# l646773422/h264-lab

Measured on AMD Instinct MI355X. Metric: 1080p macroblocks/sec, higher is better.
Workload: dtype u8

## Files before the change

h264-lab_amd/csrc/enc_kernels.h:

```cpp
#ifndef H264E_ENC_KERNELS_H
#define H264E_ENC_KERNELS_H

#include "wave.h"
#include "tables.h"
#include "h264e_dev.h"

#define MV_NA H264E_MV_NA
#define NNZ_NA 64
#define AV_T 1
#define AV_L 2
#define AV_TL 4
#define AV_TR 8
#define QMODE_I4 2
#define QMODE_INTER 8
#define QMODE_I16 9
#define QMODE_CHROMA 5
#define QD_RND 6
#define QD_THR1 10
#define QD_THR2 18
#define MUL_LAMBDA(x, l) ((x)*(l) >> 4)

DEV int mvx(mv32 v) { return (int16_t)(v & 0xffff); }
DEV int mvy(mv32 v) { return (int16_t)((uint32_t)v >> 16); }
DEV mv32 mvmk(int x, int y) { return (mv32)(((uint32_t)y << 16) | ((uint32_t)x & 0xffff)); }
DEV mv32 mvadd(mv32 a, mv32 b) { return mvmk(mvx(a) + mvx(b), mvy(a) + mvy(b)); }
DEV mv32 mvsub(mv32 a, mv32 b) { return mvmk(mvx(a) - mvx(b), mvy(a) - mvy(b)); }
DEV mv32 mvround(mv32 a) { return mvmk((mvx(a) + 1) & ~3, (mvy(a) + 1) & ~3); }

struct qblk_t { int16_t qv[16]; int16_t dq[16]; };

struct RowTask
{
    int slice_type, qp, speed, no_deblock, narrow, nslices, frame_slot;
    const uint8_t *in[3];
    int in_stride[3];
    const uint8_t *ref[3];
    uint8_t *dec[3];
    const int *dep_progress;
    mv32 clusters[2];
    const mv32 *clusters_per_mb;
};
DEV RowTask rowtask_load(const h264e_frame_task_t &T)
{
    RowTask t;
    t.slice_type = uni(T.slice_type); t.qp = uni(T.qp); t.speed = uni(T.speed); t.no_deblock = uni(T.no_deblock); t.narrow = uni(T.narrow);
    t.nslices = uni(T.nslices); t.frame_slot = uni(T.frame_slot);
    for (int c = 0; c < 3; c++) { t.in[c] = uniptr(T.in[c]); t.in_stride[c] = uni(T.in_stride[c]); t.ref[c] = uniptr(T.ref[c]); t.dec[c] = uniptr(T.dec[c]); }
    t.dep_progress = uniptr(T.dep_progress);
    t.clusters[0] = (mv32)uni(T.clusters[0]); t.clusters[1] = (mv32)uni(T.clusters[1]);
    t.clusters_per_mb = uniptr(T.clusters_per_mb);
    return t;
}


struct BitW
{
    uint64_t acc;
    int nacc;
    uint32_t pos;
    uint32_t cap;
    int overflow;
    GLOBAL_AS uint32_t *buf;
};

DEV void bw_put(BitW &b, int n, uint32_t v)
{
    n = uni(n); v = (uint32_t)uni((int)v);
    b.acc = (b.acc << n) | (uint64_t)v;
    b.nacc += n;
    if (b.nacc >= 32)
    {
        b.nacc -= 32;
        if (b.pos < b.cap) cstore32((gu8 *)(b.buf + b.pos), (uint32_t)(b.acc >> b.nacc));
        else b.overflow = 1;
        b.pos++;
        b.acc &= (1ull << b.nacc) - 1;
    }
}
DEV BitW bw_uniform(const BitW &s)
{
    BitW b;
    b.acc = (uint64_t)(uint32_t)uni((int)(uint32_t)s.acc) | ((uint64_t)(uint32_t)uni((int)(uint32_t)(s.acc >> 32)) << 32);
    b.nacc = uni(s.nacc); b.pos = (uint32_t)uni((int)s.pos); b.cap = (uint32_t)uni((int)s.cap); b.overflow = uni(s.overflow);
    b.buf = uniptr(s.buf);
    return b;
}
DEV int ue_len(uint32_t v) { return 2*(32 - clz32(v + 1)) - 1; }
DEV void bw_ue(BitW &b, uint32_t v)
{
    int n = ue_len(v);
    if (n > 32) { bw_put(b, n - 32, 0); n = 32; }
    bw_put(b, n, v + 1);
}
DEV void bw_se(BitW &b, int v) { bw_ue(b, (uint32_t)(v > 0 ? 2*v - 1 : -2*v)); }
DEV int se_len(int v) { return ue_len((uint32_t)(v > 0 ? 2*v - 1 : -2*v)); }
DEV uint32_t bw_bits(const BitW &b) { return b.pos*32u + (uint32_t)b.nacc; }


struct Plane { const gu8 *p; int w, h, stride; };

NOINLINE_DEV uint32_t ref_load4_border(const gu8 *row, int w, int x)
{
    uint32_t v = 0;
    for (int k = 0; k < 4; k++)
    {
        const int xx = imin(imax(x + k, 0), w - 1);
        v |= ((cload32(row + (xx & ~3)) >> (8*(xx & 3))) & 255u) << (8*k);
    }
    return v;
}

DEV uint64_t cload64x2(const gu8 *p) { return (uint64_t)cload32(p) | ((uint64_t)cload32(p + 4) << 32); }

DEV uint32_t ref_load4(const Plane &P, int x, int y)
{
    y = imin(imax(y, 0), P.h - 1);
    const gu8 *r = P.p + (size_t)y*P.stride;
    if (H264E_PLAIN_UNALIGNED_LOADS && x >= 0 && x + 3 < P.w) return gload32(r + x);
    if (x >= 0 && x + 7 < P.w)
    {
        const uint64_t d = cload64x2(r + (x & ~3));
        return alignbyte32((uint32_t)(d >> 32), (uint32_t)d, (unsigned)x & 3);
    }
    return ref_load4_border(r, P.w, x);
}

DEV uint32_t lds32(const uint8_t *p) { uint32_t v; memcpy(&v, p, 4); return v; }
DEV void lds32_store(uint8_t *p, uint32_t v) { memcpy(p, &v, 4); }

DEV uint32_t lds32u(const lu8 *p)
{
    const unsigned a = (unsigned)(uintptr_t)p & 3;
    const LDS_AS uint32_t *q = (const LDS_AS uint32_t *)(p - a);
    return alignbyte32(ld32_aligned(q + 1), ld32_aligned(q), a);
}

#define WIN_M 24
#define WIN_W 64
#define WIN_STRIDE 68
struct RefView
{
    Plane P; const lu8 *win; int has_win, wx0, wy0;
    const GLOBAL_AS int *dep;
    int nmbx, nmby;
    int vw, vh;
    int *far;
    int *fail;
    const int16_t *slice_row;
    int nslices;
    unsigned spin_limit;
};

DEV bool rv_inside(const RefView &V, int x0, int y0, int x1, int y1)
{
    return V.has_win && x0 >= V.wx0 && y0 >= V.wy0 && x1 < V.wx0 + V.vw && y1 < V.wy0 + V.vh;
}
DEV const lu8 *rv_ptr(const RefView &V, int x, int y) { return V.win + (y - V.wy0)*WIN_STRIDE + (x - V.wx0); }

DEV bool rv_slice_last(const RefView &V, int Y)
{
    for (int k = 1; k <= V.nslices; k++) if (V.slice_row[k] == Y + 1) return true;
    return false;
}
DEV void rv_wait_row(const RefView &V, int drow, int need)
{
    const GLOBAL_AS int *flag = V.dep + drow;
    unsigned spins = 0;
    for (;;)
    {
        const int seen = uni(dep_poll(flag));
        if (seen >= need) break;
        if (seen < 0) { if (V.fail) *V.fail = seen; break; }
        if (++spins > V.spin_limit) { if (V.fail) *V.fail = -1; break; }
        wave_nap();
    }
}
DEV void rv_wait_rect(const RefView &V, int y0, int x1, int y1)
{
    if (V.far) *V.far += 1;
    if (!V.dep) return;
    const int X = imin(imax(x1, 0), V.P.w - 1) >> 4, Ya = imin(imax(y0, 0), V.P.h - 1) >> 4, Yb = imin(imax(y1, 0), V.P.h - 1) >> 4;
    const int need = imin(X + 2, V.nmbx);
    for (int Y = Ya; Y <= Yb; Y++)
    {
        const bool last = rv_slice_last(V, Y);
        if (last) rv_wait_row(V, Y, need);
        else if (Y == Yb) rv_wait_row(V, Y + 1, need);
    }
    consumer_acquire();
}

DEV void rv_wait_rect_g(const RefView &V, int y0, int x1, int y1)
{
    if (V.far) grp_count(V.far);
    if (!V.dep) return;
    const int X = imin(imax(x1, 0), V.P.w - 1) >> 4, Ya = imin(imax(y0, 0), V.P.h - 1) >> 4, Yb = imin(imax(y1, 0), V.P.h - 1) >> 4;
    const int need = imin(X + 2, V.nmbx);
    for (int Y = Ya; Y <= Yb; Y++)
    {
        const bool last = rv_slice_last(V, Y);
        if (!last && Y != Yb) continue;
        const GLOBAL_AS int *flag = V.dep + (last ? Y : Y + 1);
        unsigned spins = 0;
        for (;;)
        {
            const int seen = dep_poll(flag);
            if (seen >= need) break;
            if (seen < 0) { if (V.fail) *V.fail = seen; break; }
            if (++spins > V.spin_limit) { if (V.fail) *V.fail = -1; break; }
            wave_nap();
        }
    }
    consumer_acquire();
}

DEV void wave_load_window(uint8_t *win, const Plane &P, int wx0, int wy0, int narrow)
{
    const int rows = narrow ? H264E_NARROW_VH : WIN_W;
    const bool interior = wx0 >= 0 && wx0 + WIN_W <= P.w;
    if (interior)
    {
        u32x4 v[4];
        WAVE_FOR(l)
        {
            const int seg = l & 3;
#pragma unroll
            for (int k = 0; k < 4; k++)
            {
                const int r = (l >> 2) + 16*k;
                if (r < rows)
                {
                    const int y = imin(imax(wy0 + r, 0), P.h - 1);
                    v[k] = cload128(P.p + (size_t)y*P.stride + wx0 + 16*seg);
                }
            }
#pragma unroll
            for (int k = 0; k < 4; k++)
            {
                const int r = (l >> 2) + 16*k;
                if (r < rows)
                {
                    uint8_t *d = win + r*WIN_STRIDE + 16*seg;
                    lds32_store(d, v[k].x); lds32_store(d + 4, v[k].y); lds32_store(d + 8, v[k].z); lds32_store(d + 12, v[k].w);
                }
            }
        }
    } else
    {
        const int nq = narrow ? (H264E_NARROW_VW + 7)/8 : WIN_W/8;
        WAVE_FOR(l)
        {
            if (l < rows)
            {
                const int y = imin(imax(wy0 + l, 0), P.h - 1);
                for (int g = 0; g < 2*nq; g++) lds32_store(win + l*WIN_STRIDE + 4*g, ref_load4(P, wx0 + 4*g, y));
            }
        }
    }
    wave_sync();
}


DEV int wave_sad_ref(const RefView &R, int x0, int y0, const uint8_t *b, int w, int h)
{
    const int g = w >> 2, n = g*h;
    if (rv_inside(R, x0, y0, x0 + w - 1, y0 + h - 1))
    {
        const lu8 *base = rv_ptr(R, x0, y0);
        return wave_sum([&](int l) -> int {
            if (l >= n) return 0;
            int r = l >> (g >> 1), c = l & (g - 1);
            return (int)sad4_u8(lds32u(base + r*WIN_STRIDE + 4*c), lds32(b + 16*r + 4*c), 0);
        });
    }
    rv_wait_rect(R, y0, x0 + w - 1, y0 + h - 1);
    return wave_sum([&](int l) -> int {
        if (l >= n) return 0;
        int r = l >> (g >> 1), c = l & (g - 1);
        return (int)sad4_u8(ref_load4(R.P, x0 + 4*c, y0 + r), lds32(b + 16*r + 4*c), 0);
    });
}

DEV int grp_sad_ref(const RefView &R, int x0, int y0, const uint8_t *b, int w, int h)
{
    const int g = w >> 2, npass = (g*h) >> 4;
    if (rv_inside(R, x0, y0, x0 + w - 1, y0 + h - 1))
    {
        const lu8 *base = rv_ptr(R, x0, y0);
        return grp_sum([&](int i) -> int {
            uint32_t s = 0;
            for (int k = 0; k < npass; k++)
            {
                const int d = i + 16*k, r = d >> (g >> 1), c = d & (g - 1);
                s = sad4_u8(lds32u(base + r*WIN_STRIDE + 4*c), lds32(b + 16*r + 4*c), s);
            }
            return (int)s;
        });
    }
    rv_wait_rect_g(R, y0, x0 + w - 1, y0 + h - 1);
    return grp_sum([&](int i) -> int {
        uint32_t s = 0;
        for (int k = 0; k < npass; k++)
        {
            const int d = i + 16*k, r = d >> (g >> 1), c = d & (g - 1);
            s = sad4_u8(ref_load4(R.P, x0 + 4*c, y0 + r), lds32(b + 16*r + 4*c), s);
        }
        return (int)s;
    });
}

DEV int grp_sad_ref_q(const RefView &R, int x0, int y0, const uint8_t *b, int sad4[4])
{
    if (rv_inside(R, x0, y0, x0 + 15, y0 + 15))
    {
        const lu8 *base = rv_ptr(R, x0, y0);
        grp_sum4([&](int i, int *v) {
            uint32_t top = 0, bot = 0;
            const int c = i & 3;
            for (int k = 0; k < 4; k++)
            {
                const int r = (i >> 2) + 4*k;
                const uint32_t s = sad4_u8(lds32u(base + r*WIN_STRIDE + 4*c), lds32(b + 16*r + 4*c), 0);
                if (k < 2) top += s; else bot += s;
            }
            v[c >> 1] = (int)top; v[2 + (c >> 1)] = (int)bot;
        }, sad4);
    } else
    {
        rv_wait_rect_g(R, y0, x0 + 15, y0 + 15);
        grp_sum4([&](int i, int *v) {
            uint32_t top = 0, bot = 0;
            const int c = i & 3;
            for (int k = 0; k < 4; k++)
            {
                const int r = (i >> 2) + 4*k;
                const uint32_t s = sad4_u8(ref_load4(R.P, x0 + 4*c, y0 + r), lds32(b + 16*r + 4*c), 0);
                if (k < 2) top += s; else bot += s;
            }
            v[c >> 1] = (int)top; v[2 + (c >> 1)] = (int)bot;
        }, sad4);
    }
    return sad4[0] + sad4[1] + sad4[2] + sad4[3];
}

DEV int wave_sad_ref_q(const RefView &R, int x0, int y0, const uint8_t *b, int sad4[4])
{
    if (rv_inside(R, x0, y0, x0 + 15, y0 + 15))
    {
        const lu8 *base = rv_ptr(R, x0, y0);
        wave_sum4([&](int l, int *v) {
            int r = l >> 2, c = l & 3;
            v[(r >> 3)*2 + (c >> 1)] = (int)sad4_u8(lds32u(base + r*WIN_STRIDE + 4*c), lds32(b + 16*r + 4*c), 0);
        }, sad4);
    } else
    {
        rv_wait_rect(R, y0, x0 + 15, y0 + 15);
        wave_sum4([&](int l, int *v) {
            int r = l >> 2, c = l & 3;
            v[(r >> 3)*2 + (c >> 1)] = (int)sad4_u8(ref_load4(R.P, x0 + 4*c, y0 + r), lds32(b + 16*r + 4*c), 0);
        }, sad4);
    }
    return sad4[0] + sad4[1] + sad4[2] + sad4[3];
}

DEV int wave_sad_lds(const uint8_t *a, const uint8_t *b, int w, int h)
{
    const int g = w >> 2, n = g*h;
    return wave_sum([&](int l) -> int {
        if (l >= n) return 0;
        int r = l >> (g >> 1), c = l & (g - 1);
        return (int)sad4_u8(lds32(a + 16*r + 4*c), lds32(b + 16*r + 4*c), 0);
    });
}

DEV int wave_sad_lds_q(const uint8_t *a, const uint8_t *b, int sad4[4])
{
    wave_sum4([&](int l, int *v) {
        int r = l >> 2, c = l & 3;
        v[(r >> 3)*2 + (c >> 1)] = (int)sad4_u8(lds32(a + 16*r + 4*c), lds32(b + 16*r + 4*c), 0);
    }, sad4);
    return sad4[0] + sad4[1] + sad4[2] + sad4[3];
}


DEV int tap6(int a, int b, int c, int d, int e, int f) { return a - 5*b + 20*c + 20*d - 5*e + f; }
DEV int tap6w(int a, int b, int c, int d, int e, int f)
{
    const int t = (c + d)*4 - (b + e);
    return (a + f) + t*4 + t;
}

template <class LD> DEV uint32_t interp_core(LD ld, int fx, int fy)
{
    if (!(fx | fy)) return ld(0, 0);
    const int pos = fx + 4*fy;
    int A[4], B[4];
    bool avg = true;
    if (fy == 0)
    {
        const uint32_t a = ld(-4, 0), b = ld(0, 0), c = ld(4, 0);
        int p[12];
#pragma unroll
        for (int k = 0; k < 4; k++) { p[k] = (int)((a >> (8*k)) & 255); p[4 + k] = (int)((b >> (8*k)) & 255); p[8 + k] = (int)((c >> (8*k)) & 255); }
#pragma unroll
        for (int i = 0; i < 4; i++)
        {
            B[i] = clip255((tap6(p[i + 2], p[i + 3], p[i + 4], p[i + 5], p[i + 6], p[i + 7]) + 16) >> 5);
            A[i] = pos == 3 ? p[5 + i] : p[4 + i];
        }
// ... 722 lines not shown
```

h264-lab_amd/csrc/enc_mb.h:

```cpp
#ifndef H264E_ENC_MB_H
#define H264E_ENC_MB_H

#include <stddef.h>
#include "enc_kernels.h"

struct GCtx { mv32 mv_left[4], mv_tl[4], mv_top[8]; };
#define GSCR_OFF(t) ((t) == 0 ? 0 : (t) == 1 ? 1024 : (t) == 2 ? 1536 : 2048)
#define GSCR_BYTES 2304

struct MbBuf
{
    alignas(16) uint8_t inp[256];
    alignas(16) uint8_t inp_c[128];
    alignas(16) uint8_t pred[256];
    alignas(4) uint8_t pix_top[36];
    alignas(4) uint8_t ptop[96];
    mv32 mv_top[8];
    uint8_t nnz_top[8];
    int8_t i4_top[4];
    uint32_t df_nz_top;
    int top_type, top_qp;
    mv32 mv[16], mvd[16];
    int type, cost, used_cand;
    mv32 mv_skip_pred;
};

struct RowLds
{
    mv32 mv_left[4], mv_tl[4];
    uint8_t nnz_left[8];
    int8_t i4_left[4];
    alignas(4) uint8_t pix_left[32];
    uint8_t pix_tl[4];
    uint32_t df_nzflag;
    mv32 df_mv[25];
    int left_type, left_qp;
    alignas(4) uint8_t strip_y[16*4];
    alignas(4) uint8_t strip_c[2][8*4];
    alignas(4) uint8_t brec[64];
    BitW bw;
    int skip_run, lead_skips, coded_any;
    int far_reads[3];
    int far_fail[3];
    int16_t slice_row[H264E_MAX_SLICES + 2];
    unsigned long long prof[4][32], prof_last[4], prof_c0, prof_w0;
    int f_noskip, f_bound, f_inter, f_decided, f_wdone, f_stop;
    int early_bound;
    int f_t3req, f_t3done;
    int f_front, d_type[2];
    int t3_sad_best, t3_lim[4];
    mv32 t3_mv_best;

    MbBuf mb[2];
    alignas(4) uint8_t trec[72];

    int8_t i4_mode[16];
    alignas(4) uint8_t bs[32];
    I4Scratch i4s;
    uint8_t nzctx[12];
    alignas(16) uint8_t pred_c[128];
    alignas(16) uint8_t i16pred[256];
    alignas(16) uint8_t tt[256];
    alignas(16) uint8_t i4rec[17*24];
    alignas(16) uint8_t ytile[20*YT_STRIDE];
    alignas(16) uint8_t ctile[2][10*CT_STRIDE];
    alignas(16) qblk_t qy[16];
    qblk_t qu[4], qv[4];
    int16_t dcy[16], dcu[4], dcv[4], lev_dcy[16], lev_dcu[4], lev_dcv[4];

    CavlcTab cavlc;
    DfTab dftab;
    int qconst[6];
    uint16_t qdat[2][42];

    mv32 part_mv[4][4], part_mvd[4][4];
    GCtx gctx[4];
    int gcost[4], gnum[4];
    alignas(16) uint8_t win[WIN_W*WIN_STRIDE + 16];
    alignas(16) uint8_t skip_pred[256];
    alignas(16) uint8_t skip_pred_c[128];
    alignas(16) uint8_t gtest[4][256];
    alignas(16) uint8_t gscr[GSCR_BYTES];

};
#define ROWLDS_INTRA_BYTES offsetof(RowLds, part_mv)

struct MbCtx
{
    const h264e_geom_t *G;
    int speed, slice_type;
    mv32 clu[2];
    const mv32 *clu_per_mb;
    Plane ref[3];
    RefView rv;
    gu8 *dec[3];
    int x, y, num, avail, type, cost, i16_mode, cropped, used_cand;
    int slice_top;
    mv32 mv_skip_pred;
    unsigned nz_mask;
    int qp;
    int lambda_mv, lambda_q4, skip_thr, skip_thr_i4, lambda_i4, lambda_i16;
};

struct rect_t { int x0, y0, x1, y1; };

DEV int in_rect(mv32 v, const rect_t &r) { return mvy(v) >= r.y0 && mvy(v) <= r.y1 && mvx(v) >= r.x0 && mvx(v) <= r.x1; }
DEV mv32 clip_rect(mv32 v, const rect_t &r) { return mvmk(imin(imax(mvx(v), r.x0), r.x1), imin(imax(mvy(v), r.y0), r.y1)); }
DEV mv32 mb_abs(const MbCtx &m, mv32 v) { return mvadd(v, mvmk(m.x*64, m.y*64)); }
DEV int mv_cost(const MbCtx &m, mv32 v, mv32 pred)
{
    return MUL_LAMBDA(se_len(mvx(v) - mvx(pred)) + se_len(mvy(v) - mvy(pred)), m.lambda_mv);
}
DEV rect_t mv_limit(const MbCtx &m) { rect_t r = { m.G->lim_x0, m.G->lim_y0, m.G->lim_x1, m.G->lim_y1 }; return r; }
DEV rect_t mv_qlimit(const MbCtx &m) { rect_t r = { m.G->lim_x0 + 16, m.G->lim_y0 + 16, m.G->lim_x1 - 16, m.G->lim_y1 - 16 }; return r; }


DEV int med3(int a, int b, int c) { return imax(imin(imax(a, b), c), imin(a, b)); }

DEV void mvp_put_arr(mv32 *mv_left, mv32 *mv_tl, mv32 *mv_top, int x, int y, int w, int h, mv32 mv)
{
    mv_tl[y] = mv_top[x + w - 1];
    for (int i = 1; i < h; i++) mv_tl[y + i] = mv;
    for (int i = 0; i < h; i++) mv_left[y + i] = mv;
    for (int i = 0; i < w; i++) mv_top[x + i] = mv;
}
DEV void mvp_put(RowLds &L, MbBuf &B, int x, int y, int w, int h, mv32 mv) { mvp_put_arr(L.mv_left, L.mv_tl, B.mv_top, x, y, w, h, mv); }

DEV mv32 mvp_get_arr(const mv32 *mv_left, const mv32 *mv_tl, const mv32 *mv_top, int flag, int x, int y, int w, int h)
{
    int type = 1;
    mv32 a = mv_left[y], b = mv_top[x], c = mv_top[x + w], d = mv_tl[y], ret = 0;
    if (!x)
    {
        if (!(flag & AV_L)) a = MV_NA;
        if (!(flag & AV_TL)) d = MV_NA;
    }
    if (!y)
    {
        if (!(flag & AV_T))
        {
            b = MV_NA;
            if (x + w < 4) c = MV_NA;
            if (x > 0) d = MV_NA;
        }
        if (!(flag & AV_TL) && !x) d = MV_NA;
        if (!(flag & AV_TR) && x + w == 4) c = MV_NA;
    }
    if (x + w == 4 && (!(flag & AV_TR) || y)) c = d;
#define OK(v) ((v) != MV_NA)
    if (OK(a) && !OK(b) && !OK(c)) type = 2;
    else if (!OK(a) && OK(b) && !OK(c)) type = 3;
    else if (!OK(a) && !OK(b) && OK(c)) type = 4;
    if (w == 2 && h == 4)
    {
        if (x == 0) { if (OK(a)) type = 2; } else { if (OK(c)) type = 4; }
    } else if (w == 4 && h == 2)
    {
        if (y == 0) { if (OK(b)) type = 3; } else { if (OK(a)) type = 2; }
    }
    if (type == 2) { if (OK(a)) ret = a; }
    else if (type == 3) { if (OK(b)) ret = b; }
    else if (type == 4) { if (OK(c)) ret = c; }
    else if (!(OK(b) || OK(c))) { if (OK(a)) ret = a; }
    else
    {
        if (!OK(a)) a = 0;
        if (!OK(b)) b = 0;
        if (!OK(c)) c = 0;
        ret = mvmk(med3(mvx(a), mvx(b), mvx(c)), med3(mvy(a), mvy(b), mvy(c)));
    }
#undef OK
    return ret;
}
DEV mv32 mvp_get(const RowLds &L, const MbBuf &B, const MbCtx &m, int x, int y, int w, int h) { return (mv32)uni(mvp_get_arr(L.mv_left, L.mv_tl, B.mv_top, m.avail, x, y, w, h)); }


DEV void set_range(mv32 &pnt, rect_t &range, const rect_t &limit, int mby_q)
{
    rect_t r = limit;
    r.y0 = (int16_t)imax(r.y0, mby_q - 63*4);
    r.y1 = (int16_t)imin(r.y1, mby_q + 63*4);
    pnt = clip_rect(pnt, r);
    mv32 tl = clip_rect(mvadd(pnt, mvmk(-32*4, -32*4)), r), br = clip_rect(mvadd(pnt, mvmk(32*4, 32*4)), r);
    range.x0 = mvx(tl); range.y0 = mvy(tl); range.x1 = mvx(br); range.y1 = mvy(br);
}

DEV int diamond_g(RowLds &L, const MbBuf &B, const MbCtx &m, int px, int py, mv32 &mv, const rect_t &range, mv32 mv_pred, int min_sad, int w, int h, uint8_t *dst, uint8_t *scr)
{
    const RefView &R = m.rv;
    const uint8_t *b = B.inp + 16*py + px;
    int c0, c1, c2, c3, p0, p1, p2, p3;
#define DX(d) ((d) == 0 ? 4 : (d) == 1 ? -4 : 0)
#define DY(d) ((d) == 2 ? 4 : (d) == 3 ? -4 : 0)
#define SEL4(d, a0, a1, a2, a3) ((d) == 0 ? (a0) : (d) == 1 ? (a1) : (d) == 2 ? (a2) : (a3))
    int cost;
    mv32 v;
    const int g = w >> 2, npass = (g*h) >> 4;
    for (;;)
// ... 754 lines not shown
```

h264-lab_amd/csrc/enc_row.h:

```cpp
#ifndef H264E_ENC_ROW_H
#define H264E_ENC_ROW_H

#include "enc_mb.h"

#define GEOM_WIDE 0
#define GEOM_NARROW 1
#define GEOM_INTRA 2

struct ChainG
{
    GLOBAL_AS h264e_mbbottom_t *bottom;
    GLOBAL_AS h264e_mbpend_t *pend;
    GLOBAL_AS int *progress;
    GLOBAL_AS uint32_t *rowbits;
    GLOBAL_AS h264e_rowmeta_t *rowmeta;
    GLOBAL_AS h264e_mbrec_t *mbrec;
    GLOBAL_AS uint8_t *arena;
    uint32_t arena_cap;
    GLOBAL_AS uint8_t *nal_arena;
    uint32_t nal_cap;
    GLOBAL_AS uint32_t *cursor;
    GLOBAL_AS h264e_frameout_t *fout;
    GLOBAL_AS int *far_reads;
    unsigned long long *prof;
};
DEV ChainG chain_view(const h264e_chain_dev_t &C)
{
    ChainG g;
    g.bottom = (GLOBAL_AS h264e_mbbottom_t *)C.bottom; g.pend = (GLOBAL_AS h264e_mbpend_t *)C.pend; g.progress = (GLOBAL_AS int *)C.progress;
    g.rowbits = (GLOBAL_AS uint32_t *)C.rowbits; g.rowmeta = (GLOBAL_AS h264e_rowmeta_t *)C.rowmeta;
    g.mbrec = (GLOBAL_AS h264e_mbrec_t *)C.mbrec; g.arena = (GLOBAL_AS uint8_t *)C.arena; g.arena_cap = C.arena_cap; g.nal_arena = (GLOBAL_AS uint8_t *)C.nal_arena; g.nal_cap = C.nal_cap;
    g.cursor = (GLOBAL_AS uint32_t *)C.cursor; g.fout = (GLOBAL_AS h264e_frameout_t *)C.fout; g.far_reads = (GLOBAL_AS int *)C.far_reads; g.prof = C.prof;
    return g;
}

DEV void row_begin(RowLds &L, const h264e_geom_t &G, const ChainG &C, const h264e_frame_task_t &T, int row)
{
    WAVE_FOR(l)
    {
        if (l < 4) { L.mv_left[l] = 0; L.mv_tl[l] = 0; L.i4_left[l] = -1; L.pix_tl[l] = 0; }
        if (l < 8) L.nnz_left[l] = NNZ_NA;
        if (l < 32) L.pix_left[l] = 0;
        if (l < 25) L.df_mv[l] = 0;
        L.strip_y[l] = 0;
        L.strip_c[l >> 5][l & 31] = 0;
    }
    L.df_nzflag = 0;
    L.left_type = 0;
    L.left_qp = T.qp;
    L.bw.acc = 0; L.bw.nacc = 0; L.bw.pos = 0; L.bw.overflow = 0;
    L.bw.cap = (uint32_t)G.row_words;
    L.bw.buf = C.rowbits + (size_t)row*G.row_words;
    L.skip_run = 0; L.lead_skips = 0; L.coded_any = 0; L.far_reads[0] = L.far_reads[1] = L.far_reads[2] = 0; L.far_fail[0] = L.far_fail[1] = L.far_fail[2] = 0;
    L.f_noskip = L.f_bound = L.f_inter = L.f_decided = L.f_wdone = L.f_stop = 0; L.early_bound = 0; L.f_t3req = L.f_t3done = L.f_front = 0;
    WAVE_FOR(l) { if (l <= H264E_MAX_SLICES) L.slice_row[l] = l <= T.nslices ? T.slice_row[l] : (int16_t)0x7fff; }
    WAVE_FOR(l)
    {
        for (int k = l; k < 84; k += 64) L.qdat[k/42][k%42] = T.qdat[k/42][k%42];
    }
    cavlc_tab_load(L.cavlc);
    df_tab_load(L.dftab);
    L.qconst[0] = k_lambda_mv_q4[T.qp]; L.qconst[1] = k_lambda_q4[T.qp]; L.qconst[2] = k_skip_thr_inter[T.qp];
    L.qconst[3] = k_skip_thr_i4x4[T.qp]; L.qconst[4] = k_lambda_i4_q4[T.qp]; L.qconst[5] = k_lambda_i16_q4[T.qp];
    for (int i = 0; i < 32; i++) L.prof[0][i] = L.prof[1][i] = L.prof[2][i] = L.prof[3][i] = 0;
    L.prof_last[0] = L.prof_last[1] = 0;
    PROF_ROW_BEGIN(L);
    wave_sync();
    PROF_ROW_SYNC(L);
}

#define LOAD_TOP_ALL 0
#define LOAD_TOP_MV 1
#define LOAD_TOP_REST 2
template <int PART> DEV void load_top(RowLds &L, MbBuf &B, const h264e_geom_t &G, const GLOBAL_AS h264e_mbbottom_t *above, const GLOBAL_AS h264e_mbpend_t *pend_above, int x, int have_top)
{
    if (PART == LOAD_TOP_MV)
    {
        WAVE_FOR(l)
        {
            if (l < 4) B.mv_top[l] = have_top ? (mv32)cload32((const gu8 *)(above + x) + 32 + 4*l) : 0;
            else if (l == 4) B.mv_top[4] = (have_top && x + 1 < G.nmbx) ? (mv32)cload32((const gu8 *)(above + x + 1) + 32) : 0;
        }
        wave_sync();
        return;
    }
    if (have_top)
    {
        WAVE_FOR(l)
        {
            if (l < 16) lds32_store(L.trec + 4*l, cload32((const gu8 *)(above + x) + 4*l));
            else if (l == 16) lds32_store(L.trec + 64, x + 1 < G.nmbx ? cload32((const gu8 *)(above + x + 1)) : 0u);
            else if (l == 17) lds32_store(L.trec + 68, x + 1 < G.nmbx ? cload32((const gu8 *)(above + x + 1) + 32) : 0u);
            else if (l >= 32 && l < 56) lds32_store(B.ptop + 4*(l - 32), cload32((const gu8 *)(pend_above + x) + 4*(l - 32)));
        }
        wave_sync();
        WAVE_FOR(l)
        {
            if (l < 8) lds32_store(B.pix_top + 4*l, lds32(L.trec + 4*l));
            else if (l < 12) { if (PART == LOAD_TOP_ALL) B.mv_top[l - 8] = (mv32)lds32(L.trec + 32 + 4*(l - 8)); }
            else if (l < 20) B.nnz_top[l - 12] = L.trec[48 + l - 12];
            else if (l < 24) B.i4_top[l - 20] = (int8_t)L.trec[56 + l - 20];
            else if (l == 24) { B.df_nz_top = L.trec[60]; B.top_type = (int8_t)L.trec[61]; B.top_qp = L.trec[62]; }
            else if (l == 25) lds32_store(B.pix_top + 32, lds32(L.trec + 64));
            else if (l == 26) { if (PART == LOAD_TOP_ALL) B.mv_top[4] = (mv32)lds32(L.trec + 68); }
        }
    } else
    {
        WAVE_FOR(l)
        {
            if (l < 36) B.pix_top[l] = 0;
            if (l < 5 && PART == LOAD_TOP_ALL) B.mv_top[l] = 0;
            if (l < 8) B.nnz_top[l] = NNZ_NA;
            if (l < 4) B.i4_top[l] = -1;
            if (l == 0) { B.df_nz_top = 0; B.top_type = 0; B.top_qp = 0; }
        }
    }
    wave_sync();
}

DEV void load_input(MbBuf &B, const h264e_geom_t &G, const RowTask &T, int mbx, int mby)
{
    const bool inside = (mbx + 1)*16 <= G.width && (mby + 1)*16 <= G.height;
    WAVE_FOR(l)
    {
        {
            int r = l >> 2, c = l & 3, yy = imin(mby*16 + r, G.height - 1);
            const gu8 *p = (const gu8 *)T.in[0] + (size_t)yy*T.in_stride[0];
            uint32_t v = 0;
            if (inside) v = gload32(p + mbx*16 + 4*c);
            else for (int k = 0; k < 4; k++) v |= (uint32_t)p[imin(mbx*16 + 4*c + k, G.width - 1)] << (8*k);
            lds32_store(B.inp + 16*r + 4*c, v);
        }
        if (l < 32)
        {
            int pl = l >> 4, r = (l >> 1) & 7, c = l & 1, yy = imin(mby*8 + r, G.height/2 - 1);
            const gu8 *p = (const gu8 *)(pl ? T.in[2] : T.in[1]) + (size_t)yy*(pl ? T.in_stride[2] : T.in_stride[1]);
            uint32_t v = 0;
            if (inside) v = gload32(p + mbx*8 + 4*c);
            else for (int k = 0; k < 4; k++) v |= (uint32_t)p[imin(mbx*8 + 4*c + k, G.width/2 - 1)] << (8*k);
            lds32_store(B.inp_c + 16*r + 8*pl + 4*c, v);
        }
    }
    wave_sync();
}

template <int GEOM> DEV void row_prefetch(RowLds &L, const h264e_geom_t &G, const RowTask &T, int row, int x)
{
    load_input(L.mb[x & 1], G, T, x, row);
    if (GEOM != GEOM_INTRA && T.slice_type == 0)
    {
        Plane P;
        P.p = (const gu8 *)T.ref[0]; P.w = G.W; P.h = G.H; P.stride = G.W;
        wave_load_window(L.win, P, x*16 - WIN_M, row*16 - WIN_M, T.narrow);
    }
}

template <int GEOM> DEV void mb_ctx_init(MbCtx &m, RowLds &L, const h264e_geom_t &G, const RowTask &T, int row, int x, int row0, int side)
{
    const bool have_top = row > row0;
    m.G = &G;
    m.speed = T.speed; m.slice_type = T.slice_type; m.clu[0] = T.clusters[0]; m.clu[1] = T.clusters[1]; m.clu_per_mb = T.clusters_per_mb;
    for (int c = 0; c < 3; c++)
    {
        m.ref[c].p = (const gu8 *)T.ref[c];
        m.ref[c].w = G.W >> (c ? 1 : 0); m.ref[c].h = G.H >> (c ? 1 : 0); m.ref[c].stride = m.ref[c].w;
        m.dec[c] = (gu8 *)T.dec[c];
    }
    m.x = x; m.y = row; m.num = row*G.nmbx + x;
    m.avail = (have_top ? AV_T : 0) | (have_top && x != G.nmbx - 1 ? AV_TR : 0) | (x > 0 ? AV_L : 0) | (have_top && x > 0 ? AV_TL : 0);
    m.slice_top = !have_top;
    m.cropped = G.cropping && ((x + 1)*16 > G.width || (row + 1)*16 > G.height);
    m.type = 0; m.cost = 0x7FFFFFFF; m.i16_mode = 0; m.used_cand = 0; m.mv_skip_pred = 0; m.nz_mask = 0;
    m.qp = T.qp;
    m.lambda_mv = uni(L.qconst[0]); m.lambda_q4 = uni(L.qconst[1]); m.skip_thr = uni(L.qconst[2]);
    m.skip_thr_i4 = uni(L.qconst[3]); m.lambda_i4 = uni(L.qconst[4]); m.lambda_i16 = uni(L.qconst[5]);
    m.rv.dep = (const GLOBAL_AS int *)T.dep_progress; m.rv.nmbx = G.nmbx; m.rv.nmby = G.nmby;
    m.rv.P = m.ref[0]; m.rv.win = (const lu8 *)L.win; m.rv.has_win = GEOM != GEOM_INTRA && T.slice_type == 0; m.rv.wx0 = x*16 - WIN_M; m.rv.wy0 = row*16 - WIN_M;
    m.rv.vw = GEOM == GEOM_NARROW ? H264E_NARROW_VW : WIN_W; m.rv.vh = GEOM == GEOM_NARROW ? H264E_NARROW_VH : WIN_W; m.rv.far = &L.far_reads[side]; m.rv.fail = &L.far_fail[side]; m.rv.slice_row = L.slice_row; m.rv.nslices = T.nslices; m.rv.spin_limit = G.spin_limit;
}

struct NoSignals { DEVM void noskip() const {} DEVM void bound(int) const {} DEVM bool helper() const { return false; } DEVM void t3_request(mv32, int, const rect_t &) const {} DEVM bool t3_wait() const { return true; } };
template <int GEOM, class SIG> DEV void mb_search(RowLds &L, MbBuf &B, const h264e_geom_t &G, const RowTask &T, int row, int x, int row0, SIG sig)
{
    MbCtx m;
    mb_ctx_init<GEOM>(m, L, G, T, row, x, row0, 0);
    STAMP(L, 1);
    if (GEOM != GEOM_INTRA && T.slice_type == 0) inter_choose(L, B, m, sig);
    STAMP(L, 7);
    B.type = m.type; B.cost = m.cost; B.used_cand = m.used_cand; B.mv_skip_pred = m.mv_skip_pred;
    wave_sync();
}

struct InterIsThere
{
    DEVM bool ready() const { return true; }
    DEVM bool wait_noskip_or_ready() const { return true; }
    DEVM bool wait_bound_or_ready() const { return true; }
    DEVM bool wait_ready() const { return true; }
    DEVM int early_bound() const { return 0x7fffffff; }
    DEVM bool before_decide() const { return true; }
};

template <class P> DEV bool mb_intra_decide(RowLds &L, MbBuf &B, MbCtx &m, const RowTask &T, P pol)
{
    bool have = pol.ready();
    if (!have)
    {
        if (!pol.wait_noskip_or_ready()) return false;
        have = pol.ready();
    }
    STAMP(L, 15);
    if (have) { m.type = uni(B.type); m.cost = uni(B.cost); }
    if (m.type >= 0)
    {
        const int cost16 = intra16_cost(L, B, m);
        STAMP(L, 8);
        int cost4 = I4_LOST, bnd = imin(m.cost, cost16);
        unsigned nz4 = 0;
        if (!have && !pol.wait_bound_or_ready()) return false;
#ifdef H264E_ABLATE
        if (H264E_ABLATE != 2)
#endif
        if (T.speed < 2 || T.slice_type != 0)
            cost4 = intra4_choose(L, B, m, [&]() -> int {
                if (!have)
                {
                    if (pol.ready()) { have = true; bnd = imin(bnd, uni(B.cost)); }
                    else bnd = imin(bnd, pol.early_bound());
                }
                return bnd;
            }, nz4);
        STAMP(L, 9);
        if (!pol.wait_ready()) return false;
        STAMP(L, 16);
        m.type = uni(B.type); m.cost = uni(B.cost);
        if (!pol.before_decide()) return false;
        if (m.type >= 0) intra_merge(L, B, m, cost16, cost4, nz4);
    } else if (!pol.before_decide()) return false;
    m.used_cand = uni(B.used_cand); m.mv_skip_pred = (mv32)uni(B.mv_skip_pred);
    mb_decide(L, B, m);
    return true;
}

struct NoHook { DEVM void operator()() const {} };
template <int GEOM, class HOOK> DEV void mb_recon_front(RowLds &L, MbBuf &B, MbCtx &m, const h264e_geom_t &G, const ChainG &C, const RowTask &T, int row, int x, int row0, int row1, HOOK after_prediction)
{
    if (GEOM == GEOM_INTRA || m.type >= 5) wave_pred_chroma(L.pred_c, L.pix_left + 16, B.pix_top + 16, m.avail, m.i16_mode);
    else predict_chroma_inter(B, m, L.pred_c);
    after_prediction();

    STAMP(L, 10);
    BitW bw = bw_uniform(L.bw);
    mb_write(L, B, m, bw);
    L.bw = bw;
    STAMP(L, 11);

    {
        GLOBAL_AS h264e_mbrec_t *rec = C.mbrec + (size_t)T.frame_slot*G.nmb + m.num;
        const uint32_t mv0 = m.type < 5 ? (uint32_t)B.mv[0] : 0u;
        const uint64_t w = (uint64_t)mv0 | ((uint64_t)(uint8_t)(int8_t)m.type << 32) | ((uint64_t)(m.used_cand & 255) << 40);
        cstore64((gu8 *)rec, w);
    }

    uint8_t *ty = L.ytile + 4*YT_STRIDE + 4;
    uint8_t *tc0 = L.ctile[0] + 2*CT_STRIDE + 2, *tc1 = L.ctile[1] + 2*CT_STRIDE + 2;
    WAVE_FOR(l)
    {
        if (l < 16)
        {
            L.pix_left[l] = ty[YT_STRIDE*l + 15];
            L.brec[l] = ty[YT_STRIDE*15 + l];
        } else if (l < 32)
        {
            int pl = (l >> 3) & 1, i = l & 7;
            const uint8_t *t = pl ? tc1 : tc0;
            L.pix_left[16 + 8*pl + i] = t[CT_STRIDE*i + 7];
            L.brec[16 + 8*pl + i] = t[CT_STRIDE*7 + i];
        } else if (l < 35)
        {
            int c = l - 32;
            L.pix_tl[c] = B.pix_top[c == 0 ? 15 : 15 + 8*c];
        }
    }
    wave_sync();

}

template <int GEOM> DEV void mb_recon_back(RowLds &L, MbBuf &B, MbCtx &m, const h264e_geom_t &G, const ChainG &C, const RowTask &T, int row, int x, int row0, int row1)
{
    const bool have_top = row > row0;
    GLOBAL_AS h264e_mbbottom_t *rowrec = C.bottom + (size_t)row*G.nmbx;
    uint8_t *ty = L.ytile + 4*YT_STRIDE + 4;
    uint8_t *tc0 = L.ctile[0] + 2*CT_STRIDE + 2, *tc1 = L.ctile[1] + 2*CT_STRIDE + 2;
    const int W = G.W, Wc = G.W >> 1;
    gu8 *dy = m.dec[0] + (size_t)(row*16)*W + x*16;
    gu8 *du = m.dec[1] + (size_t)(row*8)*Wc + x*8, *dv = m.dec[2] + (size_t)(row*8)*Wc + x*8;
    GLOBAL_AS h264e_mbpend_t *pend_row = C.pend + (size_t)row*G.nmbx;
    const bool direct = T.no_deblock || row == row1 - 1;
    if (!T.no_deblock)
    {
        df_strength(L, m, B.top_type);
        WAVE_FOR(l)
        {
            if (l < 16) lds32_store(L.ytile + (4 + l)*YT_STRIDE, lds32(L.strip_y + 4*l));
            else if (l < 32)
            {
                int pl = (l >> 3) & 1, i = l & 7;
                uint8_t *t = L.ctile[pl] + (2 + i)*CT_STRIDE;
                t[0] = L.strip_c[pl][4*i + 2]; t[1] = L.strip_c[pl][4*i + 3];
            } else if (l < 48)
            {
                int r = (l - 32) >> 2, c = l & 3;
                uint32_t v = 0;
                if (have_top) v = lds32(B.ptop + 16*r + 4*c);
                lds32_store(L.ytile + r*YT_STRIDE + 4 + 4*c, v);
            } else if (l < 56)
            {
                int pl = (l >> 2) & 1, r = (l >> 1) & 1, c = l & 1;
                uint32_t v = 0;
                if (have_top) v = lds32(B.ptop + 64 + 16*pl + 8*r + 4*c);
                memcpy(L.ctile[pl] + r*CT_STRIDE + 2 + 4*c, &v, 4);
            }
        }
        wave_sync();
        wave_deblock(L.ytile, L.ctile[0], L.ctile[1], L.bs, T.qp, L.left_qp, B.top_qp, L.dftab);
    }
    WAVE_FOR(l)
    {
        if (l < 32)
        {
// ... 463 lines not shown
```

h264-lab_amd/csrc/enc_selftest.h:

```cpp
#ifndef H264E_ENC_SELFTEST_H
#define H264E_ENC_SELFTEST_H
#include "enc_row.h"

struct StageLds
{
    alignas(16) uint8_t win[WIN_W*WIN_STRIDE + 16];
    alignas(16) uint8_t a[256], b[256], o[256];
    alignas(16) qblk_t q[16];
    alignas(4) int16_t dc[16], lev[16], coef[16];
    alignas(4) uint16_t qdat[42];
    CavlcTab ct;
    I4Scratch i4s;
    DfTab df;
    alignas(16) uint8_t yt[20*YT_STRIDE];
    alignas(16) uint8_t ctile[2][10*CT_STRIDE];
    alignas(4) uint8_t bs[32];
    alignas(4) uint8_t nb[5*24];
};
#define STAGE_IN_MAX (96*96 + 256)
#define STAGE_NARGS 24
#define STAGE_OUT_MAX (16 + 16*64 + 32 + 32 + 256)
DEV void stage_selftest(StageLds &S, RowLds &L, int stage, const GLOBAL_AS uint8_t *in, const int *args, GLOBAL_AS uint8_t *out)
{
    int a[STAGE_NARGS];
    for (int i = 0; i < STAGE_NARGS; i++) a[i] = uni(args[i]);
    Plane P = { (const gu8 *)in, 64, 64, 64 };
    RefView R;
    R.P = P; R.win = (const lu8 *)S.win; R.has_win = 0; R.wx0 = 0; R.wy0 = 0; R.dep = 0; R.nmbx = 4; R.nmby = 4; R.vw = WIN_W; R.vh = WIN_W;
    R.far = 0; R.fail = 0; R.slice_row = 0; R.nslices = 0; R.spin_limit = 0;
    GLOBAL_AS int32_t *oi = (GLOBAL_AS int32_t *)out;
    if (stage == 1 || stage == 2)
    {
        const int x = a[0], y = a[1], window = stage == 1 ? a[2] : a[6];
        if (window) { R.has_win = 1; R.wx0 = x - WIN_M; R.wy0 = y - WIN_M; wave_load_window(S.win, P, R.wx0, R.wy0, 0); wave_sync(); }
        if (stage == 1)
        {
            int s4[4];
            WAVE_FOR(l) { lds32_store(S.b + 4*l, gload32((const gu8 *)in + 4096 + 4*l)); }
            wave_sync();
            const int tot = wave_sad_ref_q(R, x, y, S.b, s4);
            if (wave_lane() == 0) { oi[0] = s4[0]; oi[1] = s4[1]; oi[2] = s4[2]; oi[3] = s4[3]; oi[4] = tot; }
        } else
        {
            WAVE_FOR(l) { lds32_store(S.o + 4*l, 0u); }
            wave_sync();
            wave_interp_luma(R, 0, 0, mvmk(4*x + a[4], 4*y + a[5]), a[2], a[3], S.o);
            wave_sync();
            WAVE_FOR(l) { gstore32((gu8 *)out + 4*l, lds32(S.o + 4*l)); }
        }
    } else if (stage == 3)
    {
        WAVE_FOR(l) { lds32_store(S.o + 4*l, 0u); }
        wave_sync();
        wave_interp_chroma(R, P, P, 0, 0, mvmk(8*a[0] + a[4], 8*a[1] + a[5]), a[2], a[3], S.o);
        wave_sync();
        WAVE_FOR(l) { gstore32((gu8 *)out + 4*l, lds32(S.o + 4*l)); }
    } else if (stage == 4)
    {
        const int mode = a[0], side = mode >> 1;
        WAVE_FOR(l)
        {
            lds32_store(S.a + 4*l, gload32((const gu8 *)in + 4*l));
            lds32_store(S.b + 4*l, gload32((const gu8 *)in + 256 + 4*l));
            if (l < 21) lds32_store((uint8_t *)S.qdat + 4*l, gload32((const gu8 *)in + 512 + 4*l));
            if (l < 8) { lds32_store((uint8_t *)S.dc + 4*l, 0u); lds32_store((uint8_t *)S.lev + 4*l, 0u); }
            for (int k = l; k < 256; k += 64) lds32_store((uint8_t *)S.q + 4*k, 0u);
        }
        wave_sync();
        unsigned nz = 0;
        int dcflag = 0;
        WAVE_FOR(l) { lds32_store(S.o + 4*l, lds32(S.b + 4*l)); }
        wave_sync();
        if (mode == QMODE_INTER) nz = wave_xform_quant_recon<QMODE_INTER>(S.a, S.b, S.o, 16, S.q, S.dc, S.lev, S.qdat, (int *)0);
        else if (mode == QMODE_I16) nz = wave_xform_quant_recon<QMODE_I16>(S.a, S.b, S.o, 16, S.q, S.dc, S.lev, S.qdat, (int *)0);
        else if (mode == QMODE_CHROMA) nz = wave_xform_quant_recon<QMODE_CHROMA>(S.a, S.b, S.o, 16, S.q, S.dc, S.lev, S.qdat, &dcflag);
        else nz = i4_block_code(i4q_make(S.qdat), S.a, S.b, S.o, 16, S.q);
        wave_sync();
        WAVE_FOR(l)
        {
            for (int k = l; k < 256; k += 64) gstore32((gu8 *)out + 8 + 4*k, lds32((const uint8_t *)S.q + 4*k));
            if (l < 8) { gstore32((gu8 *)out + 8 + 1024 + 4*l, lds32((const uint8_t *)S.dc + 4*l)); gstore32((gu8 *)out + 8 + 1056 + 4*l, lds32((const uint8_t *)S.lev + 4*l)); }
        }
        wave_sync();
        WAVE_FOR(l) { gstore32((gu8 *)out + 8 + 1088 + 4*l, lds32(S.o + 4*l)); }
        if (wave_lane() == 0) { oi[0] = (int32_t)nz; oi[1] = dcflag; }
        (void)side;
    } else if (stage == 5)
    {
        cavlc_tab_load(S.ct);
        WAVE_FOR(l) { if (l < 8) lds32_store((uint8_t *)S.coef + 4*l, gload32((const gu8 *)in + 4*l)); }
        wave_sync();
        BitW b;
        b.acc = 0; b.nacc = 0; b.pos = 0; b.cap = 60; b.overflow = 0; b.buf = (GLOBAL_AS uint32_t *)(out + 8);
        const int nnz = cavlc_block(b, S.ct, S.coef, a[0], a[1], a[2]);
        const uint32_t nbits = bw_bits(b);
        if (b.nacc) bw_put(b, 32 - b.nacc, 0);
        if (wave_lane() == 0) { oi[0] = nnz; oi[1] = (int32_t)nbits; }
    } else if (stage == 6)
    {
        WAVE_FOR(l)
        {
            if (l < 13)
            {
                const uint8_t e = in[l];
                if (l < 4) S.nb[24*(4 - l) + 3] = e;
                else S.nb[3 + (l - 4)] = e;
            }
            if (l < 16) lds32_store(S.a + 4*l, gload32((const gu8 *)in + 16 + 4*l));
            if (l < 16) lds32_store(S.o + 4*l, 0u);
        }
        wave_sync();
        const int res = wave_i4_choose(S.a, S.o, a[0], S.nb + 24 + 4, a[1], a[2], S.i4s, i4_lanes_make(24));
        wave_sync();
        WAVE_FOR(l) { if (l < 16) gstore32((gu8 *)out + 8 + 4*l, lds32(S.o + 4*l)); }
        if (wave_lane() == 0) { oi[0] = res & 15; oi[1] = res >> 4; }
    } else if (stage == 7)
    {
        const int ny = 20*YT_STRIDE, nc = 10*CT_STRIDE;
        df_tab_load(S.df);
        WAVE_FOR(l)
        {
            for (int k = l; k < ny; k += 64) S.yt[k] = in[k];
            for (int k = l; k < nc; k += 64) { S.ctile[0][k] = in[ny + k]; S.ctile[1][k] = in[ny + nc + k]; }
            if (l < 32) S.bs[l] = in[ny + 2*nc + l];
        }
        wave_sync();
        wave_deblock(S.yt, S.ctile[0], S.ctile[1], S.bs, a[0], a[1], a[2], S.df);
        wave_sync();
        WAVE_FOR(l)
        {
            for (int k = l; k < ny; k += 64) out[k] = S.yt[k];
            for (int k = l; k < nc; k += 64) { out[ny + k] = S.ctile[0][k]; out[ny + nc + k] = S.ctile[1][k]; }
        }
    } else if (stage == 8)
    {
        h264e_geom_t Gs;
        MbCtx m;
        Plane P8 = { (const gu8 *)in, 96, 96, 96 };
        Gs.width = Gs.W = 96; Gs.height = Gs.H = 96; Gs.nmbx = Gs.nmby = 6; Gs.nmb = 36; Gs.cropping = 0;
        Gs.lim_x0 = a[15]; Gs.lim_y0 = a[16]; Gs.lim_x1 = a[17]; Gs.lim_y1 = a[18];
        m.G = &Gs; m.speed = a[10]; m.slice_type = 0; m.x = 2; m.y = 2; m.num = 14; m.qp = a[9];
        m.lambda_mv = k_lambda_mv_q4[a[9]];
        m.rv = R; m.rv.P = P8; m.rv.nmbx = 6; m.rv.nmby = 6;
        if (a[19]) { m.rv.has_win = 1; m.rv.win = (const lu8 *)L.win; m.rv.wx0 = 32 - WIN_M; m.rv.wy0 = 32 - WIN_M; wave_load_window(L.win, P8, m.rv.wx0, m.rv.wy0, 0); }
        WAVE_FOR(l) { lds32_store(L.mb[0].inp + 4*l, gload32((const gu8 *)in + 96*96 + 4*l)); lds32_store(L.gtest[0] + 4*l, 0u); }
        wave_sync();
        const rect_t range = { a[11], a[12], a[13], a[14] };
        GRP_EACH(grp)
        {
            if (grp == (a[20] & 3))
            {
                mv32 mv = mvmk(a[4], a[5]);
                const int cost = diamond_g(L, L.mb[0], m, a[0], a[1], mv, range, mvmk(a[6], a[7]), a[8], a[2], a[3], L.gtest[0] + 16*a[1] + a[0], L.gscr);
                L.gcost[0] = cost; L.gcost[1] = mvx(mv); L.gcost[2] = mvy(mv);
            }
        }
        wave_sync();
        WAVE_FOR(l) { gstore32((gu8 *)out + 16 + 4*l, lds32(L.gtest[0] + 4*l)); }
        if (wave_lane() == 0) { oi[0] = L.gcost[0]; oi[1] = L.gcost[1]; oi[2] = L.gcost[2]; }
    }
}

DEV uint32_t sv_h32(uint32_t a)
{
    a ^= a >> 16; a *= 0x7feb352du; a ^= a >> 15; a *= 0x846ca68bu; a ^= a >> 16;
    return a;
}
DEV int sv_lattice(int32_t ix, int32_t iy, uint32_t seed) { return (int)(sv_h32((uint32_t)ix*0x9E3779B1u ^ (uint32_t)iy*0x85EBCA77u ^ seed) & 255); }
DEV int sv_tex(int32_t X, int32_t Y, uint32_t seed, int lg)
{
    int32_t c = 1 << lg, ix = X >> lg, iy = Y >> lg, fx = X & (c - 1), fy = Y & (c - 1);
    int32_t a = sv_lattice(ix, iy, seed), b = sv_lattice(ix + 1, iy, seed), cc = sv_lattice(ix, iy + 1, seed), d = sv_lattice(ix + 1, iy + 1, seed);
    int32_t top = a*(c - fx) + b*fx, bot = cc*(c - fx) + d*fx;
    return (top*(c - fy) + bot*fy + (1 << (2*lg - 1))) >> (2*lg);
}
DEV uint8_t sv_sample(int w, int h, int t, uint32_t seed, int idx)
{
    const int32_t OFF = 1 << 20;
    if (idx < w*h)
    {
        int x = idx % w, y = idx / w, fw = w/8 > 32 ? w/8 : 32, fh = h/6 > 32 ? h/6 : 32;
        int fx0 = (w/2 + ((10*t) >> 2)) % (w - fw), fy0 = h/3, v;
        if (x >= fx0 && x < fx0 + fw && y >= fy0 && y < fy0 + fh) v = sv_tex(4*x - 10*t + OFF, 4*y + OFF, seed + 1, 5);
        else v = (sv_tex(4*x + 5*t + OFF, 4*y + 3*t + OFF, seed, 6)*3 >> 2) + 32;
        v += (int)(sv_h32((uint32_t)x ^ ((uint32_t)y << 12) ^ ((uint32_t)t << 24) ^ (uint32_t)(seed*7919u)) % 5) - 2;
        return (uint8_t)clip255(v);
    }
    idx -= w*h;
    const int cw = w/2, ch = h/2, pl = idx >= cw*ch;
    if (pl) idx -= cw*ch;
    int x = idx % cw, y = idx / cw;
    if (!pl) return (uint8_t)(128 + ((sv_tex(8*x + 5*t + OFF, 8*y + 3*t + OFF, seed + 2, 7) - 128) >> 2));
    return (uint8_t)(128 - ((sv_tex(8*x + 5*t + OFF, 8*y + 3*t + OFF, seed + 3, 7) - 128) >> 3));
}

#endif
```

Before: 13.74 million.

## Slide the reference search window as a ring buffer instead of reloading it

The LDS motion-search window becomes a circular buffer with a mirrored tail (stride widened to 120), addressed from an origin of wx0 & 60. When the previous macroblock's window is still resident, only the newly exposed 16-pixel column strip is loaded rather than the whole 64x64 window, which cuts global-memory traffic per macroblock. The profiling arrays are also moved under a compile flag, which shrinks LDS use. In exchange every store writes twice near the wrap point, LDS use per row grows, and correctness now depends on the ring-origin arithmetic matching rv_ptr.

```diff
diff --git a/h264-lab_amd/csrc/enc_kernels.h b/h264-lab_amd/csrc/enc_kernels.h
--- a/h264-lab_amd/csrc/enc_kernels.h
+++ b/h264-lab_amd/csrc/enc_kernels.h
@@ -137,7 +137,7 @@
 
 #define WIN_M 24
 #define WIN_W 64
-#define WIN_STRIDE 68
+#define WIN_STRIDE 120
 struct RefView
 {
     Plane P; const lu8 *win; int has_win, wx0, wy0;
@@ -156,6 +156,13 @@
     return V.has_win && x0 >= V.wx0 && y0 >= V.wy0 && x1 < V.wx0 + V.vw && y1 < V.wy0 + V.vh;
 }
 DEV const lu8 *rv_ptr(const RefView &V, int x, int y) { return V.win + (y - V.wy0)*WIN_STRIDE + (x - V.wx0); }
+DEV int win_org(int wx0) { return wx0 & 60; }
+DEV void win_store4(uint8_t *row, int pos, uint32_t v)
+{
+    pos &= 63;
+    lds32_store(row + pos, v);
+    if (pos < WIN_STRIDE - 64) lds32_store(row + pos + 64, v);
+}
 
 DEV bool rv_slice_last(const RefView &V, int Y)
 {
@@ -218,6 +225,7 @@
 {
     const int rows = narrow ? H264E_NARROW_VH : WIN_W;
     const bool interior = wx0 >= 0 && wx0 + WIN_W <= P.w;
+    const int org = win_org(wx0);
     if (interior)
     {
         u32x4 v[4];
@@ -240,8 +248,9 @@
                 const int r = (l >> 2) + 16*k;
                 if (r < rows)
                 {
-                    uint8_t *d = win + r*WIN_STRIDE + 16*seg;
-                    lds32_store(d, v[k].x); lds32_store(d + 4, v[k].y); lds32_store(d + 8, v[k].z); lds32_store(d + 12, v[k].w);
+                    uint8_t *d = win + r*WIN_STRIDE;
+                    const int pos = org + 16*seg;
+                    win_store4(d, pos, v[k].x); win_store4(d, pos + 4, v[k].y); win_store4(d, pos + 8, v[k].z); win_store4(d, pos + 12, v[k].w);
                 }
             }
         }
@@ -253,8 +262,31 @@
             if (l < rows)
             {
                 const int y = imin(imax(wy0 + l, 0), P.h - 1);
-                for (int g = 0; g < 2*nq; g++) lds32_store(win + l*WIN_STRIDE + 4*g, ref_load4(P, wx0 + 4*g, y));
-            }
+                for (int g = 0; g < 2*nq; g++) win_store4(win + l*WIN_STRIDE, org + 4*g, ref_load4(P, wx0 + 4*g, y));
+            }
+        }
+    }
+    wave_sync();
+}
+
+template <bool NARROW> DEV void wave_slide_window(uint8_t *win, const Plane &P, int wx0, int wy0)
+{
+    constexpr int rows = NARROW ? H264E_NARROW_VH : WIN_W;
+    constexpr int rel = NARROW ? (H264E_NARROW_VW - 16) & ~3 : WIN_W - 16;
+    static_assert(!NARROW || rel + 20 >= H264E_NARROW_VW, "the narrow strip is five dwords");
+    const int pos = win_org(wx0) + rel;
+    WAVE_FOR(l)
+    {
+        if (l < rows)
+        {
+            const int y = imin(imax(wy0 + l, 0), P.h - 1);
+            const gu8 *s = P.p + (size_t)y*P.stride + wx0 + rel;
+            const u32x4 v = cload128(s);
+            uint32_t t = 0;
+            if (NARROW) t = cload32(s + 16);
+            uint8_t *d = win + l*WIN_STRIDE;
+            win_store4(d, pos, v.x); win_store4(d, pos + 4, v.y); win_store4(d, pos + 8, v.z); win_store4(d, pos + 12, v.w);
+            if (NARROW) win_store4(d, pos + 16, t);
         }
     }
     wave_sync();
diff --git a/h264-lab_amd/csrc/enc_mb.h b/h264-lab_amd/csrc/enc_mb.h
--- a/h264-lab_amd/csrc/enc_mb.h
+++ b/h264-lab_amd/csrc/enc_mb.h
@@ -42,8 +42,11 @@
     int skip_run, lead_skips, coded_any;
     int far_reads[3];
     int far_fail[3];
+    int win_x;
     int16_t slice_row[H264E_MAX_SLICES + 2];
+#ifdef H264E_STAMPS
     unsigned long long prof[4][32], prof_last[4], prof_c0, prof_w0;
+#endif
     int f_noskip, f_bound, f_inter, f_decided, f_wdone, f_stop;
     int early_bound;
     int f_t3req, f_t3done;
diff --git a/h264-lab_amd/csrc/enc_row.h b/h264-lab_amd/csrc/enc_row.h
--- a/h264-lab_amd/csrc/enc_row.h
+++ b/h264-lab_amd/csrc/enc_row.h
@@ -62,8 +62,11 @@
     df_tab_load(L.dftab);
     L.qconst[0] = k_lambda_mv_q4[T.qp]; L.qconst[1] = k_lambda_q4[T.qp]; L.qconst[2] = k_skip_thr_inter[T.qp];
     L.qconst[3] = k_skip_thr_i4x4[T.qp]; L.qconst[4] = k_lambda_i4_q4[T.qp]; L.qconst[5] = k_lambda_i16_q4[T.qp];
+    L.win_x = -2;
+#ifdef H264E_STAMPS
     for (int i = 0; i < 32; i++) L.prof[0][i] = L.prof[1][i] = L.prof[2][i] = L.prof[3][i] = 0;
     L.prof_last[0] = L.prof_last[1] = 0;
+#endif
     PROF_ROW_BEGIN(L);
     wave_sync();
     PROF_ROW_SYNC(L);
@@ -151,7 +154,10 @@
     {
         Plane P;
         P.p = (const gu8 *)T.ref[0]; P.w = G.W; P.h = G.H; P.stride = G.W;
-        wave_load_window(L.win, P, x*16 - WIN_M, row*16 - WIN_M, T.narrow);
+        const int wx0 = x*16 - WIN_M;
+        if (uni(L.win_x) == x - 1 && wx0 - 16 >= 0 && wx0 + WIN_W <= P.w) wave_slide_window<GEOM == GEOM_NARROW>(L.win, P, wx0, row*16 - WIN_M);
+        else wave_load_window(L.win, P, wx0, row*16 - WIN_M, T.narrow);
+        L.win_x = x;
     }
 }
 
@@ -175,7 +181,7 @@
     m.lambda_mv = uni(L.qconst[0]); m.lambda_q4 = uni(L.qconst[1]); m.skip_thr = uni(L.qconst[2]);
     m.skip_thr_i4 = uni(L.qconst[3]); m.lambda_i4 = uni(L.qconst[4]); m.lambda_i16 = uni(L.qconst[5]);
     m.rv.dep = (const GLOBAL_AS int *)T.dep_progress; m.rv.nmbx = G.nmbx; m.rv.nmby = G.nmby;
-    m.rv.P = m.ref[0]; m.rv.win = (const lu8 *)L.win; m.rv.has_win = GEOM != GEOM_INTRA && T.slice_type == 0; m.rv.wx0 = x*16 - WIN_M; m.rv.wy0 = row*16 - WIN_M;
+    m.rv.P = m.ref[0]; m.rv.win = (const lu8 *)L.win + win_org(x*16 - WIN_M); m.rv.has_win = GEOM != GEOM_INTRA && T.slice_type == 0; m.rv.wx0 = x*16 - WIN_M; m.rv.wy0 = row*16 - WIN_M;
     m.rv.vw = GEOM == GEOM_NARROW ? H264E_NARROW_VW : WIN_W; m.rv.vh = GEOM == GEOM_NARROW ? H264E_NARROW_VH : WIN_W; m.rv.far = &L.far_reads[side]; m.rv.fail = &L.far_fail[side]; m.rv.slice_row = L.slice_row; m.rv.nslices = T.nslices; m.rv.spin_limit = G.spin_limit;
 }
 
diff --git a/h264-lab_amd/csrc/enc_selftest.h b/h264-lab_amd/csrc/enc_selftest.h
--- a/h264-lab_amd/csrc/enc_selftest.h
+++ b/h264-lab_amd/csrc/enc_selftest.h
@@ -32,7 +32,7 @@
     if (stage == 1 || stage == 2)
     {
         const int x = a[0], y = a[1], window = stage == 1 ? a[2] : a[6];
-        if (window) { R.has_win = 1; R.wx0 = x - WIN_M; R.wy0 = y - WIN_M; wave_load_window(S.win, P, R.wx0, R.wy0, 0); wave_sync(); }
+        if (window) { R.has_win = 1; R.wx0 = x - WIN_M; R.wy0 = y - WIN_M; R.win = (const lu8 *)S.win + win_org(R.wx0); wave_load_window(S.win, P, R.wx0, R.wy0, 0); wave_sync(); }
         if (stage == 1)
         {
             int s4[4];
@@ -142,7 +142,7 @@
         m.G = &Gs; m.speed = a[10]; m.slice_type = 0; m.x = 2; m.y = 2; m.num = 14; m.qp = a[9];
         m.lambda_mv = k_lambda_mv_q4[a[9]];
         m.rv = R; m.rv.P = P8; m.rv.nmbx = 6; m.rv.nmby = 6;
-        if (a[19]) { m.rv.has_win = 1; m.rv.win = (const lu8 *)L.win; m.rv.wx0 = 32 - WIN_M; m.rv.wy0 = 32 - WIN_M; wave_load_window(L.win, P8, m.rv.wx0, m.rv.wy0, 0); }
+        if (a[19]) { m.rv.has_win = 1; m.rv.wx0 = 32 - WIN_M; m.rv.win = (const lu8 *)L.win + win_org(m.rv.wx0); m.rv.wy0 = 32 - WIN_M; wave_load_window(L.win, P8, m.rv.wx0, m.rv.wy0, 0); }
         WAVE_FOR(l) { lds32_store(L.mb[0].inp + 4*l, gload32((const gu8 *)in + 96*96 + 4*l)); lds32_store(L.gtest[0] + 4*l, 0u); }
         wave_sync();
         const rect_t range = { a[11], a[12], a[13], a[14] };
```

New measurement: 13.90 million (median of 6 runs). 1.01x the previous value.
